# surftemp/cae_tools

Hardware: AMD Instinct MI355X
Metric: train images/sec (16x16->256x256, batch 64) (higher is better)
Workload: dtype f32

## Files before the change

cae_tools_amd/csrc/engine.hip:

```cpp
#include <hip/hip_runtime.h>

#include <dlfcn.h>

#include <algorithm>
#include <cmath>
#include <cstdio>
#include <cstdlib>
#include <cstring>
#include <map>
#include <string>
#include <tuple>
#include <vector>

#include "cae_hip.h"
#include "kernels_generic.h"
#include "kernels_s2.h"
#include "kernels_last.h"
#include "kernels_rows.h"
#include "kernels_gemm.h"
#include "kernels_igemm.h"
#include "kernels_ctlds.h"
#include "kernels_head.h"
#include "dp_comm.h"
#include "kernels_ctbwd.h"
#include "trunk_api.h"
#include "engine_host.h"

namespace cae {
template __global__ void k_ct_fwd_lds<3, 3>(CtFwd);
template __global__ void k_s2_fwd_rows<8, 4, 1, 2>(S2FwdRows);
template __global__ void k_s2_fwd_rows<4, 2, 2, 1>(S2FwdRows);
template __global__ void k_s2_last_fused<2, 1, 4, 4, 4, true, true>(S2Last);
template __global__ void k_s2_bwd_rows<4, 4, 2, 3, 3, 2, 1, 3>(S2Rows);
template __global__ void k_s2_bwd_rows<8, 2, 4, 3, 3, 4, 2, 1>(S2Rows);
}

using namespace cae;
using namespace cae_internal;

namespace cae_internal {
int ctbwd_launch(const void* args, size_t bytes, unsigned gx, unsigned gy, unsigned gz, size_t lds, hipStream_t s);
}

namespace {
thread_local std::string g_err;
}

void cae_detail_set_error(const char* msg) { g_err = msg; }

namespace {

constexpr float kBnEps = 1e-5f;
constexpr float kBnMomentum = 0.1f;
constexpr int kLossSlots = 1 << 16;

// ... 39 lines not shown
    int64_t ws_need = 0;

    float *params = nullptr, *grads = nullptr, *m = nullptr, *v = nullptr, *bufs = nullptr;
    char* ws = nullptr;
    hipStream_t stream = nullptr;
    Hyper hp{1e-3, 0.9, 0.999, 1e-8, 1e-5};
    const float* ds_x[2] = {nullptr, nullptr};
    const float* ds_t[2] = {nullptr, nullptr};
    int64_t ds_n[2] = {0, 0};
    bool graph_mode = true;
    bool lr_stale = true;
    long long captures = 0;
    bool capture_only = false;
    bool use_s2 = true;
    bool variational = false;
    int64_t off_vz = 0, off_vgz = 0, off_zlast = 0;
    cae_internal::TrunkHooks hooks{nullptr, nullptr, nullptr};
    bool gather_fwd = false;
    int ctbwd_mask = 0;
    int ctbwd_auto = 0;
    int64_t off_xbatch = 0;
    bool x_published = false;
    AdamConv0 c0_pending{};
    bool profiling = false;
    struct ProfRec { const char* name; int layer; double bytes; hipEvent_t e0, e1; };
    std::vector<ProfRec> prof;
    std::map<std::tuple<int, int, int, int, const void*, int, int, int, int, int>, hipGraphExec_t> graphs;

    int dp_world = 0, dp_rank = 0;
    RcclApi::comm_t dp_comm = nullptr;
    hipStream_t comm_stream = nullptr;
    hipEvent_t ev_fork = nullptr, ev_join = nullptr;
    bool dp_graph_ok = true;
    bool dp_overlap = true;
    std::vector<int> sync_order;
    size_t sync_pos = 0;
    int64_t bucket_split = 0;

    StepState* state() const { return reinterpret_cast<StepState*>(ws + off_state); }
    double* losses() const { return reinterpret_cast<double*>(ws + off_losses); }
    double* gradacc() const { return reinterpret_cast<double*>(ws + off_gradacc); }
    double* sgacc() const { return reinterpret_cast<double*>(ws + off_sgacc); }
    ShardSegs shard_segs() const {
        ShardSegs r = segs;
        r.base = sgacc();
        return r;
// ... 385 lines not shown
}

void rows_fwd_launch(const ConvLayer& L, S2FwdRows a, hipStream_t s) {
    const RowsPick p = choose_rows_fwd(L);
    a.QH = (L.hout + 1) / 2;
    if (L.cin == 4) rows_fwd_go<4, 2, 2>(a, p.lw, s);
    else rows_fwd_go<8, 4, 1>(a, p.lw, s);
}

bool last_fused_ok(const cae_engine* e, const ConvLayer& L) {
    return s2_eligible(e, L) && L.cin * L.cout * L.kh * L.kw <= 72 && L.sh_b >= 0;
}

constexpr int kLastHB = 4;

struct LastPick { bool vec4, bn; };

int last_strips(const ConvLayer& L) {
    const int qw = (L.wout + 1) / 2;
    const int wmax = L.win > qw - 1 ? L.win : qw - 1;
    return (wmax + kLastStripPx - 1) / kLastStripPx;
}

LastPick choose_last(const ConvLayer& L, bool bn_in) { return LastPick{last_strips(L) == 1 && (L.wout & 3) == 0, bn_in}; }

template <int CIN, int COUT, int KH, int KW>
bool last_fused_launch(S2Last a, LastPick p, hipStream_t s) {
    if constexpr (CIN * COUT * KH * KW <= 72) {
        a.QH = (a.OH + 1) / 2;
        a.QW = (a.OW + 1) / 2;
        const int wmax = a.W > a.QW - 1 ? a.W : a.QW - 1, hmax = a.H > a.QH - 1 ? a.H : a.QH - 1;
        a.strips = (wmax + kLastStripPx - 1) / kLastStripPx;
        a.bands = (hmax + kLastHB - 1) / kLastHB;
        a.total = a.B * a.strips * a.bands;
        const dim3 grid((a.total + 3) / 4);
        if (p.vec4 && p.bn) hipLaunchKernelGGL((k_s2_last_fused<CIN, COUT, KH, KW, kLastHB, true, true>), grid, dim3(256), 0, s, a);
        else if (p.bn) hipLaunchKernelGGL((k_s2_last_fused<CIN, COUT, KH, KW, kLastHB, false, true>), grid, dim3(256), 0, s, a);
        else hipLaunchKernelGGL((k_s2_last_fused<CIN, COUT, KH, KW, kLastHB, false, false>), grid, dim3(256), 0, s, a);
        return true;
    }
    return false;
}

bool last_fused_dispatch(const ConvLayer& L, const S2Last& a, hipStream_t s) {
    const LastPick p = choose_last(L, a.bn_in.mode != BN_NONE);
#define ONE(CI, CO, KH_, KW_) \
    if (L.cin == CI && L.cout == CO && L.kh == KH_ && L.kw == KW_) return last_fused_launch<CI, CO, KH_, KW_>(a, p, s);
#define PAIR(CI, CO) S2_KERNELS(ONE, CI, CO)
    S2_SHAPES(PAIR)
#undef PAIR
#undef ONE
    return false;
}

template <class K>
void head_lds_attr(K kernel, size_t bytes) {
    static size_t granted = 64 * 1024;
    if (bytes > granted) {
// ... 255 lines not shown
    DF_CT_LDS,
    DF_IG,
    DF_UP
};
enum DecBwdK {
    DB_FUSED_LAST,
    DB_ROWS,
    DB_S2,
    DB_CT_LDS,
    DB_IG,
    DB_GENERIC
};

int s2_fwd_epi(const cae_engine* e, int l, bool train, bool external_loss) {
    if (l + 1 < (int)e->dec.size()) return train ? S2_RAW_STATS : S2_RAW;
    if (external_loss) return S2_RAW;
    return train ? S2_SIGMSE : S2_SIGOUT;
}

bool rows_ok(const cae_engine* e, const ConvLayer& L, int l) {
    return l + 1 < (int)e->dec.size() && l > 0 && e->dec[l - 1].has_bn && rows_bwd_ok(e, L);
}

DecFwdK choose_dec_fwd(const cae_engine* e, const ConvLayer& L, int l, int B, bool train, bool external_loss) {
    const bool last = l + 1 == (int)e->dec.size();
    if (last && train && !external_loss && last_fused_ok(e, L)) return DF_FUSED_LAST;
    if (rows_ok(e, L, l)) return DF_ROWS;
    if (s2_eligible(e, L)) return DF_S2;
    if (e->use_s2 && !last && L.stride == 2 && L.kh <= 4 && L.kw <= 4) {
        CtFwd c;
        int waves = 0;
        size_t lds = 0;
        return ct_fwd_plan(e, B, L, l, c, waves, lds) ? DF_CT_LDS : DF_IG;
    }
    return DF_UP;
}

DecBwdK choose_dec_bwd(const cae_engine* e, const ConvLayer& L, int l, int B, bool external_loss) {
    const bool last = l + 1 == (int)e->dec.size();
    if (last && !external_loss && last_fused_ok(e, L)) return DB_FUSED_LAST;
    if (rows_ok(e, L, l)) return DB_ROWS;
    if (s2_eligible(e, L)) return DB_S2;
    if (e->use_s2) {
        CtBwdPlan p;
        return ct_bwd_plan(e, B, L, l, p) ? DB_CT_LDS : DB_IG;
    }
// ... 34 lines not shown
        hipLaunchKernelGGL(k_narrow_range, dim3(grid1(hi - lo)), dim3(256), 0, on, (long long)lo, (long long)hi, e->grads,
                           e->shard_segs(), narrow_tail(e, false, 0));
    }
    if (int rc = dp_allreduce_grads(e, lo, hi, on)) return rc;
    if (overlap) HIP_TRY(hipEventRecord(e->ev_join, e->comm_stream));
    return CAE_OK;
}

int dp_finish_step(cae_engine* e, const StepArgs& a) {
    hipStream_t s = e->stream;
    const int64_t lo = 0, hi = dp_single_collective(e, a) ? e->tab.n_param : e->bucket_split;
    {
        ProfScope _p(e, "dp_narrow_bucket1", 0, 12.0 * (hi - lo));
        hipLaunchKernelGGL(k_narrow_range, dim3(grid1(hi - lo > 0 ? hi - lo : 1)), dim3(256), 0, s, (long long)lo, (long long)hi,
                           e->grads, e->shard_segs(), narrow_tail(e, true, a.inc()));
    }
    if (dp_overlap(e, a)) HIP_TRY(hipStreamWaitEvent(s, e->ev_join, 0));
    if (int rc = dp_allreduce_grads(e, lo, hi, s)) return rc;
    StepTail none;
    memset(&none, 0, sizeof none);
    ProfScope _p(e, "adam", 0, 28.0 * e->tab.n_param);
    hipLaunchKernelGGL(k_adam, dim3(grid1(e->tab.n_param)), dim3(256), 0, s, (long long)e->tab.n_param, e->params,
                       (const float*)e->grads, e->m, e->v, e->hp, (const StepState*)e->state(), e->shard_segs(), none, 0,
                       std::log(e->hp.beta1), std::log(e->hp.beta2), AdamConv0{});
    return CAE_OK;
}

int launch_forward(cae_engine* e, const StepArgs& a) {
    hipStream_t s = e->stream;
    const int B = a.batch;
    const StepState* st = e->state();
    const int act_mode = a.train ? BN_BATCH : BN_RUNNING;

    HeadArgs head;
    size_t head_lds = 0;
    const bool fused_head = a.part == 0 && head_plan(e, a, head, head_lds);
    if (fused_head) {
        head.x = a.x_direct ? a.x_direct : e->ds_x[a.which];
        head.perm = a.x_direct ? nullptr : a.perm;
        head.use_cursor = a.x_direct ? 0 : 1;
        head.bump_adam = a.train ? 1 : 0;
        const int T = (e->fc[3].nout + 15) / 16;
        double bytes = 0;
        for (auto& L : e->enc) bytes += f4((double)B * (L.in_elems() + L.out_elems()));
        for (int i = 0; i < 4; i++) bytes += f4((double)B * (e->fc[i].nin + e->fc[i].nout) + (double)e->fc[i].nin * e->fc[i].nout);
        head_lds_attr(k_head_fwd, head_lds);
        e->x_published = false;
// ... 245 lines not shown
            memset(&f, 0, sizeof f);
            f.B = B; f.H = L.hin; f.W = L.win; f.OH = L.hout; f.OW = L.wout;
            f.in = ain.p;
            f.w = e->params + L.w_off;
            f.bias = e->params + L.b_off;
            f.target = e->ds_t[a.which];
            f.perm = a.perm;
            f.use_cursor = a.use_cursor ? 1 : 0;
            f.st = st;
            f.losses = e->losses();
            f.inv_count = (float)(1.0 / ((double)a.global_batch * L.cout * L.hout * L.wout));
            f.bias_acc = e->sgacc() + L.sh_b;
            f.wacc = e->sgacc() + L.sh_w;
            f.acc_stride = e->segs.n;
            if (l == 0) {
                f.bn_in = bn_none();
                f.gin = e->fptr(e->fc[3].grad_off);
            } else {
                const ConvLayer& P = e->dec[l - 1];
                f.bn_in = bn_of(e, P, BN_BATCH, (double)a.bn_batch * P.hout * P.wout, 1);
                f.gin = e->fptr(P.grad_off);
                f.stats_in = e->bn_stats(P.bn_index);
            }
            ProfScope _p(e, "s2_convt_last_fused", l, f4((double)B * (L.in_elems() * 2.0 + L.out_elems())));
            if (!last_fused_dispatch(L, f, s))
                return fail(CAE_ERR_STATE, "decoder layer %d: no k_s2_last_fused kernel for the chosen variant", (int)l);
            if (l > 0)
                if (int rc = sync_bn_table(e, a, e->dec[l - 1].bn_index)) return rc;
            continue;
        }
        if (bk == DB_ROWS) {
            const ConvLayer& P = e->dec[l - 1];
            S2Rows f;
            memset(&f, 0, sizeof f);
            f.B = B; f.H = L.hin; f.W = L.win; f.OH = L.hout; f.OW = L.wout;
            f.g = gy.p; f.yout = gy.q; f.bn_out = bng;
            f.ain = ain.p; f.bn_in = bna;
            f.w = e->params + L.w_off;
            f.gin = e->fptr(P.grad_off);
            f.stats_in = e->bn_stats(P.bn_index);
            f.wacc = e->sgacc() + L.sh_w;
            f.wacc_stride = e->segs.n;
            f.bg.stats = e->bn_stats(L.bn_index);
            f.bg.gamma_acc = acc + L.gamma_off;
            f.bg.beta_acc = acc + L.beta_off;
            f.bg.C = L.cout;
            f.bg.scale = 1.0 / a.world;
// ... 403 lines not shown
        ProfScope _cal(e, "event_pair", -1, 0.0);
    }
    if (op == OP_DP_TRAIN) {
        e->sync_pos = 0;
        if (a.batch > 0) {
            int rc = launch_forward(e, a);
            if (rc) return rc;
            rc = launch_backward(e, a);
            if (rc) return rc;
        } else {
            hipLaunchKernelGGL(k_bump_adam, dim3(1), dim3(1), 0, s, e->state());
            if (a.dp_sync)
                for (int bn : e->sync_order)
                    if (int rc = sync_bn_table(e, a, bn)) return rc;
            if (int rc = dp_first_bucket(e, a)) return rc;
        }
        if (a.dp_sync && e->sync_pos != e->sync_order.size())
            return fail(CAE_ERR_STATE, "SyncBN: %zu of %zu tables all-reduced", e->sync_pos, e->sync_order.size());
        if (int rc = dp_finish_step(e, a)) return rc;
    } else if (op == OP_TRAIN || op == OP_FWDBWD) {
        StepArgs af = a;
        af.adam_follows = op == OP_TRAIN;
        memset(&e->c0_pending, 0, sizeof e->c0_pending);
        int rc = launch_forward(e, af);
        if (rc) return rc;
        rc = launch_backward(e, af);
        if (rc) return rc;
        if (op == OP_TRAIN) {
            ProfScope _p(e, "adam", 0, 32.0 * e->tab.n_param);
            AdamConv0 c0 = e->c0_pending;
            StepTail tl = step_tail_of(e, a.inc(), 1);
            int nreg = grid1(e->tab.n_param), grid = nreg;
            if (c0.on) {
                const long long skip = (long long)kStatShards * c0.C * 4;
                tl.zero_extra += skip;
                tl.zero_extra_n -= skip;
                c0.n_regular = nreg;
                grid = nreg + c0.nw;
            }
            hipLaunchKernelGGL(k_adam, dim3(grid), dim3(256), 0, s, (long long)e->tab.n_param, e->params,
                               (const float*)nullptr, e->m, e->v, e->hp, (const StepState*)e->state(), e->shard_segs(),
                               tl, 0, std::log(e->hp.beta1), std::log(e->hp.beta2), c0);
        } else {
            hipLaunchKernelGGL(k_acc_to_f32, dim3(grid1(e->tab.n_param)), dim3(256), 0, s, (long long)e->tab.n_param, e->grads,
                               e->shard_segs(), step_tail_of(e, a.inc(), 1));
        }
    } else if (op == OP_EVAL) {
        int rc = launch_forward(e, a);
        if (rc) return rc;
        if (a.use_cursor) hipLaunchKernelGGL(k_advance, dim3(1), dim3(1), 0, s, e->state(), a.inc(), 1, 0);
    } else if (op == OP_ADAM) {
        StepTail none;
        memset(&none, 0, sizeof none);
        hipLaunchKernelGGL(k_adam, dim3(grid1(e->tab.n_param)), dim3(256), 0, s, (long long)e->tab.n_param, e->params,
                           (const float*)e->grads, e->m, e->v, e->hp, (const StepState*)e->state(), e->shard_segs(),
                           none, 0, std::log(e->hp.beta1), std::log(e->hp.beta2), AdamConv0{});
    }
    HIP_TRY(hipGetLastError());
    return CAE_OK;
}

int push_lr(cae_engine* e) {
    if (!e->lr_stale || !e->ws) return CAE_OK;
    hipLaunchKernelGGL(k_set_lr, dim3(1), dim3(1), 0, e->stream, e->state(), e->hp.lr);
    HIP_TRY(hipGetLastError());
    e->lr_stale = false;
    return CAE_OK;
}

int run_op(cae_engine* e, int op, const StepArgs& a, bool cacheable) {
    if (int rc = push_lr(e)) return rc;
    if (!e->graph_mode || !cacheable || e->stream == nullptr || e->profiling)
        return e->capture_only ? CAE_OK : launch_op(e, op, a);
    auto key = std::make_tuple(op, a.which, a.batch, a.global_batch, (const void*)a.perm, a.nsteps, a.cursor_inc,
                               a.dp_sync ? 1 : 0, a.bn_batch, a.world);
    auto it = e->graphs.find(key);
    if (it == e->graphs.end()) {
        hipGraph_t graph = nullptr;
        HIP_TRY(hipStreamBeginCapture(e->stream, hipStreamCaptureModeThreadLocal));
// ... 198 lines not shown
    for (auto& L : e->dec) reg_bn(L);
    e->off_gradacc = carve(e->tab.n_param * (int64_t)sizeof(double));
    e->off_sgacc = carve((int64_t)kStatShards * (e->segs.n > 0 ? e->segs.n : 4) * (int64_t)sizeof(double));
    e->off_zero_end = carve.top;
    for (auto& L : e->enc) e->bn_saved_off[L.bn_index] = carve((int64_t)L.cout * 2 * sizeof(float));
    for (auto& L : e->dec)
        if (L.has_bn) e->bn_saved_off[L.bn_index] = carve((int64_t)L.cout * 2 * sizeof(float));
    const int64_t mb = max_batch;
    for (auto& L : e->enc) {
        L.act_off = carve(mb * L.out_elems() * 4);
        L.grad_off = carve(mb * L.out_elems() * 4);
    }
    for (int i = 0; i < 4; i++) {
        e->fc[i].act_off = carve(mb * e->fc[i].nout * 4);
        e->fc[i].grad_off = carve(mb * e->fc[i].nout * 4);
    }
    for (auto& L : e->dec) {
        if (!L.has_bn) continue;
        L.act_off = carve(mb * L.out_elems() * 4);
        L.grad_off = carve(mb * L.out_elems() * 4);
    }
    e->off_glast = carve(mb * e->dec.back().out_elems() * 4);
    e->off_xbatch = carve((mb * e->enc[0].in_elems() + e->enc[0].cout) * 4);
    if (variational) {
        e->off_vz = carve(mb * latent_size * 4);
        e->off_vgz = carve(mb * latent_size * 4);
        e->off_zlast = carve(mb * e->dec.back().out_elems() * 4);
    }
    e->ws_need = carve.top;
    for (auto& L : e->enc)
        if (L.cin > e->max_channels) e->max_channels = L.cin;
    for (auto& L : e->dec)
        if (L.cin > e->max_channels) e->max_channels = L.cin;
    if (lds_bytes(e->max_channels, e->max_channels) > 60 * 1024) {
        delete e;
        return fail(CAE_ERR_ARG, "channel count %d exceeds the LDS constant table", e->max_channels);
    }
    *out = e;
    return CAE_OK;
}

void cae_engine_destroy(cae_engine* e) {
    if (!e) return;
    e->drop_graphs();
    (void)cae_dp_shutdown(e);
    delete e;
// ... 536 lines not shown
    int n = 0;
    for (auto& r : e->prof) {
        float ms = 0.f;
        hipError_t rc = hipEventElapsedTime(&ms, r.e0, r.e1);
        if (rc == hipSuccess && out && n < capacity) {
            memset(&out[n], 0, sizeof out[n]);
            snprintf(out[n].name, sizeof out[n].name, "%s", r.name);
            out[n].layer = r.layer;
            out[n].micros = (double)ms * 1000.0;
            out[n].bytes = r.bytes;
            n++;
        }
        (void)hipEventDestroy(r.e0);
        (void)hipEventDestroy(r.e1);
    }
    e->prof.clear();
    return n;
}

int cae_debug_plan(const cae_engine* e, int batch, int train, char* out, int64_t out_bytes) {
    if (!e || !out || out_bytes < 1) return fail(CAE_ERR_ARG, "cae_debug_plan: bad argument");
    if (batch < 1 || batch > e->max_batch) return fail(CAE_ERR_ARG, "cae_debug_plan: batch %d outside 1 .. %d", batch, e->max_batch);
    const bool tr = train != 0, ext = e->variational;
    const StepArgs a{0, nullptr, batch, batch, batch, tr, true, nullptr, nullptr, false};
    std::string s;
    char line[256];
    {
        HeadArgs h;
        size_t lds = 0;
        snprintf(line, sizeof line, "head fwd=%s\n", head_plan(e, a, h, lds) ? "fused" : "layers");
        s += line;
    }
    static const char* const kEpiName[] = {"raw_stats", "sigmse", "sigout", "raw"};
    for (int l = 0; l < (int)e->dec.size(); l++) {
        const ConvLayer& L = e->dec[l];
        const int ci = L.cin, co = L.cout, kh = L.kh, kw = L.kw;
        char f[128], b[128];
        switch (choose_dec_fwd(e, L, l, batch, tr, ext)) {
            case DF_FUSED_LAST: {
                const LastPick p = choose_last(L, l > 0 && e->dec[l - 1].has_bn);
                snprintf(f, sizeof f, "last_fused<%d,%d,%d,%d> hb=%d vec4=%d bn=%d", ci, co, kh, kw, kLastHB, (int)p.vec4, (int)p.bn);
                break;
            }
            case DF_ROWS: {
                const RowsPick p = choose_rows_fwd(L);
                snprintf(f, sizeof f, "s2_fwd_rows<%d,%d,%d,%d>", ci, co, p.hb, 64 / p.lw);
                break;
            }
            case DF_S2: {
                const int epi = s2_fwd_epi(e, l, tr, ext);
                const S2FwdPick p = choose_s2_fwd(L, batch, epi);
                const char* fam = p.k == S2F_CS ? "s2_fwd_cs" : (p.k == S2F_QUAD ? "s2_fwd" : "s2_fwd2");
                snprintf(f, sizeof f, "%s<%d,%d,%d,%d,%d> epi=%s", fam, ci, co, kh, kw, p.tw, kEpiName[epi]);
                break;
            }
            case DF_CT_LDS: snprintf(f, sizeof f, "ct_fwd_lds<%d,%d>", kh, kw); break;
            case DF_IG: snprintf(f, sizeof f, "ig_fwd_s2"); break;
            case DF_UP: snprintf(f, sizeof f, "up"); break;
        }
        if (!tr) {
            snprintf(b, sizeof b, "-");
        } else {
            switch (choose_dec_bwd(e, L, l, batch, ext)) {
                case DB_FUSED_LAST: snprintf(b, sizeof b, "(fused)"); break;
// ... 387 lines not shown
    } else if (int rc = launch_forward(e, a)) {
        return rc;
    }
    HIP_TRY(hipGetLastError());
    return CAE_OK;
}

int trunk_backward(cae_engine* e, const float* x, int batch, const ShardSync& sync) {
    if (!e || !e->ws || !e->variational) return fail(CAE_ERR_STATE, "trunk_backward: not a bound trunk engine");
    StepArgs a = trunk_args(x, batch, true, sync);
    a.external_loss = true;
    if (int rc = batch == 0 ? trunk_empty_shard(e, a, false) : launch_backward(e, a)) return rc;
    if (a.ordered && e->sync_pos != e->sync_order.size())
        return fail(CAE_ERR_STATE, "SyncBN: %zu of %zu tables passed to the callback", e->sync_pos, e->sync_order.size());
    HIP_TRY(hipGetLastError());
    return CAE_OK;
}

int trunk_adam(cae_engine* e) {
    if (!e || !e->ws) return fail(CAE_ERR_STATE, "trunk_adam: not a bound engine");
    if (int rc = push_lr(e)) return rc;
    hipLaunchKernelGGL(k_adam, dim3(grid1(e->tab.n_param)), dim3(256), 0, e->stream, (long long)e->tab.n_param, e->params,
                       (const float*)nullptr, e->m, e->v, e->hp, (const StepState*)e->state(), e->shard_segs(),
                       step_tail_of(e, 0, 0), 0, std::log(e->hp.beta1), std::log(e->hp.beta2), AdamConv0{});
    HIP_TRY(hipGetLastError());
    return CAE_OK;
}

int trunk_gradients(cae_engine* e, float* out, double scale) {
    if (!e || !e->ws || !out) return fail(CAE_ERR_STATE, "trunk_gradients: bad argument");
    hipLaunchKernelGGL(k_acc_to_f32, dim3(grid1(e->tab.n_param)), dim3(256), 0, e->stream, (long long)e->tab.n_param, out, e->shard_segs(),
                       step_tail_of(e, 0, 0));
    if (scale != 1.0)
        hipLaunchKernelGGL(k_scale_f32, dim3(grid1(e->tab.n_param)), dim3(256), 0, e->stream, out, (long long)e->tab.n_param, (float)scale);
    HIP_TRY(hipGetLastError());
    return CAE_OK;
}

int trunk_adam_from(cae_engine* e, const float* grads) {
    if (!e || !e->ws || !grads) return fail(CAE_ERR_STATE, "trunk_adam_from: bad argument");
    if (int rc = push_lr(e)) return rc;
    StepTail none;
    memset(&none, 0, sizeof none);
    hipLaunchKernelGGL(k_adam, dim3(grid1(e->tab.n_param)), dim3(256), 0, e->stream, (long long)e->tab.n_param, e->params, grads, e->m, e->v,
                       e->hp, (const StepState*)e->state(), e->shard_segs(), none, 0, std::log(e->hp.beta1), std::log(e->hp.beta2),
                       AdamConv0{});
    HIP_TRY(hipGetLastError());
    return CAE_OK;
}

}
```

cae_tools_amd/csrc/kernels_generic.h:

```cpp
#pragma once
#include <hip/hip_runtime.h>
#include <stdint.h>

namespace cae {

constexpr int kStatShards = 8;

#include "acc_grid.h"

struct ShardSeg {
    long long param_off;
    int count;
    int sh_off;
};
struct ShardSegs {
    int nseg;
    int n;
    const double* base;
    ShardSeg seg[12];
};

__device__ __forceinline__ double sharded_grad(const ShardSegs& ss, long long i) {
    double g = 0.0;
    for (int s = 0; s < ss.nseg; s++) {
// ... 678 lines not shown
    float sum = 0.f, bsum = 0.f;
    for (int b = 0; b < B; b++) {
        const float gv = gout[(size_t)b * nout + o];
        sum = fmaf(gv, bn_apply(bni.mode, k, in[(size_t)b * nin + i], 0.f), sum);
        bsum += gv;
    }
    accW[idx] = (double)sum;
    if (i == 0) accB[o] = (double)bsum;
}

struct Hyper {
    double lr, beta1, beta2, eps, wd;
};

struct StepTail {
    double* zero_extra;
    long long zero_extra_n;
    double* acc_rw;
    double* shard_rw;
    StepState* st;
    int batch_inc, slot_inc;
};

__device__ __forceinline__ float consume_grad(const StepTail& tl, const ShardSegs& ss, long long i) {
    double g = tl.acc_rw[i];
    tl.acc_rw[i] = 0.0;
    for (int s = 0; s < ss.nseg; s++) {
        const long long d = i - ss.seg[s].param_off;
        if (d >= 0 && d < ss.seg[s].count) {
            double* p = tl.shard_rw + ss.seg[s].sh_off + d;
            double v[kStatShards];
#pragma unroll
            for (int sh = 0; sh < kStatShards; sh++) v[sh] = p[(size_t)sh * ss.n];
#pragma unroll
            for (int sh = 0; sh < kStatShards; sh++) {
                g += v[sh];
                p[(size_t)sh * ss.n] = 0.0;
            }
        }
    }
    return (float)g;
}

__device__ __forceinline__ void step_tail(const StepTail& tl, long long gid, long long nthreads) {
    for (long long j = gid; j < tl.zero_extra_n; j += nthreads) tl.zero_extra[j] = 0.0;
    if (gid == 0 && tl.st) {
        tl.st->batch_start += tl.batch_inc;
        tl.st->loss_slot += tl.slot_inc;
    }
}

struct AdamConv0 {
    int on, nw, C, n_regular;
    long long w_off, gamma_off, beta_off;
    ConvGeom g;
    Src small;
    BnDesc bns;
    const float* xb;
    const double* stats;
    double scale;
};
constexpr int kAdamConv0Pos = 16;

__device__ __forceinline__ void adam_conv0_body(const AdamConv0& c0, float* __restrict__ p, float* __restrict__ m,
// ... 45 lines not shown
    const float4 ks = cs4[cs];
    float sum = 0.f;
#pragma unroll
    for (int u = 0; u < kAdamConv0Pos; u++)
        if (tid + u * 256 < n) sum = fmaf(bn_apply(BN_BWD, ks, sp[u], sq[u]), lp[u], sum);
    for (int pp = tid + kAdamConv0Pos * 256; pp < n; pp += 256) {
        float a, b, c;
        fetch(pp, a, b, c);
        sum = fmaf(bn_apply(BN_BWD, ks, a, b), c, sum);
    }
    const double tot = block_sum((double)sum, red);
    if (tid == 0) {
        float gr = (float)(tot * c0.scale);
        if (h.wd != 0.0) gr = fmaf((float)h.wd, w, gr);
        mi = mi + (gr - mi) * (float)(1.0 - h.beta1);
        vi = vi * (float)h.beta2 + ((float)(1.0 - h.beta2) * gr) * gr;
        const float denom = sqrtf(vi) / corr[1] + (float)h.eps;
        p[pi] = w - corr[0] * (mi / denom);
        m[pi] = mi;
        v[pi] = vi;
    }
}

__global__ void __launch_bounds__(256) k_adam(long long n, float* __restrict__ p, const float* __restrict__ g32,
                                               float* __restrict__ m, float* __restrict__ v, Hyper h,
                                               const StepState* __restrict__ st, ShardSegs ss, StepTail tl, int t_add,
                                               double ln_b1, double ln_b2, AdamConv0 c0) {
    kernarg_warm<sizeof(Hyper) + sizeof(ShardSegs) + sizeof(StepTail) + 72 + sizeof(AdamConv0)>();
    const long long i = (long long)blockIdx.x * 256 + threadIdx.x;
    __shared__ float corr[2];
    if (c0.on && (int)blockIdx.x >= c0.n_regular) {
        __shared__ double red0[8];
        __shared__ float4 cs40[64];
        adam_conv0_body(c0, p, m, v, h, st, t_add, ln_b1, ln_b2, corr, red0, cs40);
        return;
    }
    for (long long j = i; j < tl.zero_extra_n; j += (long long)(c0.on ? c0.n_regular : (int)gridDim.x) * 256) tl.zero_extra[j] = 0.0;
    int t = 0;
    double lr = 0.0;
    if (threadIdx.x < 2) {
        optimiser_state(st, t, lr);
        t += t_add;
    }
    const bool moves_cursor = i == 0 && tl.st != nullptr;
    long long cursor = 0;
    int slot = 0;
    if (moves_cursor) {
        cursor = tl.st->batch_start;
        slot = tl.st->loss_slot;
    }
    const bool mine = i < n && !(c0.on && i >= c0.w_off && i < c0.w_off + c0.nw);
    float g = 0.f, w = 0.f, mi = 0.f, vi = 0.f;
    double gacc = 0.0, sv[kStatShards], bv[kStatShards];
    double* shp = nullptr;
    const double* bnp = nullptr;
    if (mine) {
        w = p[i];
        mi = m[i];
        vi = v[i];
        if (g32) {
            g = g32[i];
        } else {
            gacc = tl.acc_rw[i];
            for (int sg = 0; sg < ss.nseg; sg++) {
                const long long d = i - ss.seg[sg].param_off;
                if (d >= 0 && d < ss.seg[sg].count) shp = tl.shard_rw + ss.seg[sg].sh_off + d;
            }
            if (shp) {
#pragma unroll
                for (int sh = 0; sh < kStatShards; sh++) sv[sh] = shp[(size_t)sh * ss.n];
            }
            if (c0.on) {
                const long long dg = i - c0.gamma_off, db = i - c0.beta_off;
                if (dg >= 0 && dg < c0.C) bnp = c0.stats + dg * 4 + 3;
// ... 556 lines not shown
```

cae_tools_amd/csrc/kernels_last.h:

```cpp
#pragma once
#include <utility>
#include "kernels_s2.h"

namespace cae {

template <class F, int... Is>
__device__ __forceinline__ void static_for_impl(F&& f, std::integer_sequence<int, Is...>) {
    (f(std::integral_constant<int, Is>{}), ...);
}
template <int N, class F>
__device__ __forceinline__ void static_for(F&& f) {
    static_for_impl(f, std::make_integer_sequence<int, N>{});
}

struct S2Last {
    int B, H, W, OH, OW;
    int QH, QW;
    int strips, bands;
    int total;
    const float* in;
    BnDesc bn_in;
    const float* w;
    const float* bias;
    const float* target;
    const int* perm;
    int use_cursor;
    const StepState* st;
    double* losses;
    float inv_count;
    double* bias_acc;
    double* wacc;
    int acc_stride;
    float* gin;
    double* stats_in;
};

constexpr int kLastStripPx = 127;

__device__ __forceinline__ float uniform_f(float v) {
    return __builtin_bit_cast(float, __builtin_amdgcn_readfirstlane(__builtin_bit_cast(int, v)));
}
__device__ __forceinline__ float from_left(float v, float edge) {
    return __builtin_bit_cast(float, __builtin_amdgcn_update_dpp(__builtin_bit_cast(int, edge), __builtin_bit_cast(int, v), 0x138, 0xF, 0xF, false));
}
__device__ __forceinline__ float from_right(float v, float edge) {
    return __builtin_bit_cast(float, __builtin_amdgcn_update_dpp(__builtin_bit_cast(int, edge), __builtin_bit_cast(int, v), 0x130, 0xF, 0xF, false));
}

constexpr int kWsumLd = 68;
constexpr int kWsumScratch = 16 * kWsumLd;
template <int N>
__device__ __forceinline__ void wave_sums_lds(const float (&v)[N], float* scr, float* out, int lane) {
    const int row = lane >> 2, qd = lane & 3;
#pragma unroll
    for (int c0 = 0; c0 < N; c0 += 16) {
#pragma unroll
        for (int i = 0; i < 16; i++)
            if (c0 + i < N) scr[i * kWsumLd + lane] = v[c0 + i];
        const float4* p = reinterpret_cast<const float4*>(scr + row * kWsumLd + 4 * qd);
        const float4 a0 = p[0], a1 = p[4], a2 = p[8], a3 = p[12];
        float t = ((a0.x + a0.y) + (a0.z + a0.w)) + ((a1.x + a1.y) + (a1.z + a1.w)) + ((a2.x + a2.y) + (a2.z + a2.w)) +
                  ((a3.x + a3.y) + (a3.z + a3.w));
        t += dpp_f<0xB1>(t);
        t += dpp_f<0x4E>(t);
        if (qd == 0 && c0 + row < N) out[c0 + row] = t;
    }
}

template <int CIN, int COUT, int KH, int KW, int HB, bool VEC4, bool BN>
__global__ void __launch_bounds__(256) __attribute__((amdgpu_waves_per_eu(1, 2))) k_s2_last_fused(S2Last a) {
    kernarg_warm<sizeof(S2Last)>();
    constexpr int NACC = CIN * COUT * KH * KW;
    constexpr int NRED = NACC + 2 * CIN;
    constexpr int NR = HB + 1;
    static_assert(KH >= 3 && KH <= 4 && KW >= 3 && KW <= 4, "3- or 4-tap stride-2 kernels");
    __shared__ float redf[4 * NRED];
    __shared__ double redd[4 * 2 * COUT];
    __shared__ __attribute__((aligned(16))) float wscr[4 * kWsumScratch];
    __shared__ float xch[4 * CIN * 2 * 64];

    const int tid = threadIdx.x, lane = tid & 63;
    const int wv = __builtin_amdgcn_readfirstlane(tid >> 6);
    const unsigned HW = a.H * a.W, OHW = a.OH * a.OW;

    const int item = blockIdx.x * 4 + wv;
    const bool work = item < a.total;
    const int it = work ? item : 0;
    const int b = it / (a.strips * a.bands);
    const int rem = it - b * (a.strips * a.bands);
    const int band = rem / a.strips, strip = rem - band * a.strips;
    const int m0 = band * HB;
    const bool last_band = band == a.bands - 1, last_strip = strip == a.strips - 1;
// ... 303 lines not shown
        if (y < a.H) {
            const bool p0 = n0 < a.W, p1 = n0 + 1 < a.W && lane < 63;
#pragma unroll
            for (int ci = 0; ci < CIN; ci++) {
                float gv0 = carry[ci][0] + xch[(((wv + 1) * CIN + ci) * 2 + 0) * 64 + lane];
                float gv1 = carry[ci][1] + xch[(((wv + 1) * CIN + ci) * 2 + 1) * 64 + lane];
                if constexpr (BN) {
                    const float e0 = rin[HB][ci][0] - kc[ci].x, e1 = rin[HB][ci][1] - kc[ci].x;
                    gv0 = fmaf(e0, kc[ci].y, kc[ci].z) > 0.f ? gv0 : 0.f;
                    gv1 = fmaf(e1, kc[ci].y, kc[ci].z) > 0.f ? gv1 : 0.f;
                    const float s0 = p0 ? gv0 : 0.f, s1 = p1 ? gv1 : 0.f;
                    d1[ci] += s0 + s1;
                    d2[ci] = fmaf(s0, e0 * kc[ci].w, fmaf(s1, e1 * kc[ci].w, d2[ci]));
                }
                float* gp = a.gin + (size_t)(b * CIN + ci) * HW + (unsigned)y * a.W + n0;
                if (p0) {
                    gp[0] = gv0;
                    gp[p1 ? 1 : 0] = p1 ? gv1 : gv0;
                }
            }
        }
    }

    {
        float red[NRED];
#pragma unroll
        for (int i = 0; i < NACC; i++) red[i] = dw[i];
#pragma unroll
        for (int c = 0; c < CIN; c++) {
            red[NACC + 2 * c] = d1[c];
            red[NACC + 2 * c + 1] = d2[c];
        }
        wave_sums_lds<NRED>(red, wscr + wv * kWsumScratch, redf + wv * NRED, lane);
    }
#pragma unroll
    for (int co = 0; co < COUT; co++) {
        const double t1 = wave_sum_lane63((double)ls[co] * (double)a.inv_count), t2 = wave_sum_lane63((double)gs[co]);
        if (lane == 63) {
            redd[(wv * COUT + co) * 2] = t1;
            redd[(wv * COUT + co) * 2 + 1] = t2;
        }
    }
    __syncthreads();
    const int shard = blockIdx.x & (kStatShards - 1);
    for (int j = tid; j < NRED + 2 * COUT; j += 256) {
        if (j < NRED) {
            const double s = (double)redf[j] + (double)redf[NRED + j] + (double)redf[2 * NRED + j] + (double)redf[3 * NRED + j];
            if (j < NACC) {
                acc_add<ACC_GRAD>(&a.wacc[(size_t)shard * a.acc_stride + j], s);
            } else if (a.stats_in) {
                const int jj = j - NACC;
                acc_add<ACC_GRAD>(&a.stats_in[((size_t)shard * CIN + (jj >> 1)) * 4 + 2 + (jj & 1)], s);
            }
        } else {
            const int q = j - NRED, co = q >> 1, which = q & 1;
            double s = 0.0;
#pragma unroll
            for (int w = 0; w < 4; w++) s += redd[(w * COUT + co) * 2 + which];
            if (which == 0) acc_add<ACC_GRAD>(&a.losses[(size_t)loss_slot_v * kStatShards + shard], s);
            else acc_add<ACC_GRAD>(&a.bias_acc[(size_t)shard * a.acc_stride + co], s);
        }
    }
    asm volatile("" :: "v"(perm_val_v));
}

}
```

cae_tools_amd/engine.py:

```python
import ctypes as C
from collections import OrderedDict

import numpy as np
import torch

from . import _lib
from ._engine_base import TEST, TRAIN, SpecPlan, _spec_layers, _to_c, require_gpu
from ._lib import CaeError, check


class EnginePlan(SpecPlan):

    PREFIX = "cae_"

    def bn_prefixes(self):
        return [n[: -len(".running_mean")] for n in self.tensors if n.endswith(".running_mean")]

    def set_kernel_mode(self, mode):
        check(self.lib.cae_set_kernel_mode(self.handle, int(mode)))

    def kernel_plan(self, batch, train):
        buf = C.create_string_buffer(1 << 16)
        check(self.lib.cae_debug_plan(self.handle, int(batch), 1 if train else 0, buf, len(buf)))
        plan = {}
        for line in buf.value.decode().splitlines():
            (name, *fields) = line.split()
            plan[name] = dict(f.split("=", 1) for f in fields)
        return plan


class HipEngine(EnginePlan):

    def __init__(self, spec, fc_size, latent_size, max_batch, device=None, graph=True, specialised=True):
        require_gpu()
        super().__init__(spec, fc_size, latent_size, max_batch)
        self._bind(device, grads=True, buffers=True)
        check(self.lib.cae_set_graph_mode(self.handle, 1 if graph else 0))
        check(self.lib.cae_set_kernel_mode(self.handle, int(specialised) if isinstance(specialised, int) and not isinstance(specialised, bool) else (1 if specialised else 0)))
        torch.cuda.synchronize(self.device)
        self.num_batches_tracked = 0
        self.adam_steps = 0
        self._datasets = {}
        self._keep = []
        self.loss_slots = int(self.lib.cae_loss_slots(self.handle))
        self._slot = 0
        self._cursor = None
# ... 574 lines not shown
```

Baseline: 384,100.

## Write last-layer weight/bias/loss partial sums to a slab reduced inside Adam

In the fused last decoder kernel, each block now writes its weight-gradient, bias-gradient and loss partial sums to a per-block row in a double-precision slab instead of issuing sharded atomic adds. The Adam kernel gains extra blocks that reduce the slab columns and apply the update for those parameters directly, and it also accumulates the loss. This is meant to remove atomic contention on the small last-layer gradient set. The cost is extra slab memory traffic, extra Adam blocks, and a code path that only applies to single-device fused training steps.

```diff
diff --git a/cae_tools_amd/csrc/engine.hip b/cae_tools_amd/csrc/engine.hip
--- a/cae_tools_amd/csrc/engine.hip
+++ b/cae_tools_amd/csrc/engine.hip
@@ -31,6 +31,7 @@
 template __global__ void k_s2_fwd_rows<8, 4, 1, 2>(S2FwdRows);
 template __global__ void k_s2_fwd_rows<4, 2, 2, 1>(S2FwdRows);
 template __global__ void k_s2_last_fused<2, 1, 4, 4, 4, true, true>(S2Last);
+template __global__ void k_s2_last_fused<2, 1, 4, 4, 4, true, true, true>(S2Last);
 template __global__ void k_s2_bwd_rows<4, 4, 2, 3, 3, 2, 1, 3>(S2Rows);
 template __global__ void k_s2_bwd_rows<8, 2, 4, 3, 3, 4, 2, 1>(S2Rows);
 }
@@ -116,6 +117,9 @@
     int64_t off_xbatch = 0;
     bool x_published = false;
     AdamConv0 c0_pending{};
+    int64_t off_slab_last = 0;
+    int slab_last_rows = 0;
+    AdamSlab slab_pending{};
     bool profiling = false;
     struct ProfRec { const char* name; int layer; double bytes; hipEvent_t e0, e1; };
     std::vector<ProfRec> prof;
@@ -547,6 +551,13 @@
     return (wmax + kLastStripPx - 1) / kLastStripPx;
 }
 
+int last_grid(const ConvLayer& L, int B) {
+    const int qh = (L.hout + 1) / 2;
+    const int hmax = L.hin > qh - 1 ? L.hin : qh - 1;
+    const int bands = (hmax + kLastHB - 1) / kLastHB;
+    return (B * last_strips(L) * bands + 3) / 4;
+}
+
 LastPick choose_last(const ConvLayer& L, bool bn_in) { return LastPick{last_strips(L) == 1 && (L.wout & 3) == 0, bn_in}; }
 
 template <int CIN, int COUT, int KH, int KW>
@@ -559,6 +570,13 @@
         a.bands = (hmax + kLastHB - 1) / kLastHB;
         a.total = a.B * a.strips * a.bands;
         const dim3 grid((a.total + 3) / 4);
+        if (a.slab) {
+            a.slab_stride = last_slab_stride(CIN * COUT * KH * KW, COUT);
+            if (p.vec4 && p.bn) hipLaunchKernelGGL((k_s2_last_fused<CIN, COUT, KH, KW, kLastHB, true, true, true>), grid, dim3(256), 0, s, a);
+            else if (p.bn) hipLaunchKernelGGL((k_s2_last_fused<CIN, COUT, KH, KW, kLastHB, false, true, true>), grid, dim3(256), 0, s, a);
+            else hipLaunchKernelGGL((k_s2_last_fused<CIN, COUT, KH, KW, kLastHB, false, false, true>), grid, dim3(256), 0, s, a);
+            return true;
+        }
         if (p.vec4 && p.bn) hipLaunchKernelGGL((k_s2_last_fused<CIN, COUT, KH, KW, kLastHB, true, true>), grid, dim3(256), 0, s, a);
         else if (p.bn) hipLaunchKernelGGL((k_s2_last_fused<CIN, COUT, KH, KW, kLastHB, false, true>), grid, dim3(256), 0, s, a);
         else hipLaunchKernelGGL((k_s2_last_fused<CIN, COUT, KH, KW, kLastHB, false, false>), grid, dim3(256), 0, s, a);
@@ -860,6 +878,10 @@
     return l + 1 < (int)e->dec.size() && l > 0 && e->dec[l - 1].has_bn && rows_bwd_ok(e, L);
 }
 
+bool last_slab(const cae_engine* e, const StepArgs& a) {
+    return a.adam_follows && !a.syncing() && a.world == 1 && !a.dp && !a.external_loss && e->slab_last_rows > 0;
+}
+
 DecFwdK choose_dec_fwd(const cae_engine* e, const ConvLayer& L, int l, int B, bool train, bool external_loss) {
     const bool last = l + 1 == (int)e->dec.size();
     if (last && train && !external_loss && last_fused_ok(e, L)) return DF_FUSED_LAST;
@@ -940,7 +962,7 @@
     ProfScope _p(e, "adam", 0, 28.0 * e->tab.n_param);
     hipLaunchKernelGGL(k_adam, dim3(grid1(e->tab.n_param)), dim3(256), 0, s, (long long)e->tab.n_param, e->params,
                        (const float*)e->grads, e->m, e->v, e->hp, (const StepState*)e->state(), e->shard_segs(), none, 0,
-                       std::log(e->hp.beta1), std::log(e->hp.beta2), AdamConv0{});
+                       std::log(e->hp.beta1), std::log(e->hp.beta2), AdamConv0{}, AdamSlab{});
     return CAE_OK;
 }
 
@@ -1232,7 +1254,24 @@
                 f.gin = e->fptr(P.grad_off);
                 f.stats_in = e->bn_stats(P.bn_index);
             }
-            ProfScope _p(e, "s2_convt_last_fused", l, f4((double)B * (L.in_elems() * 2.0 + L.out_elems())));
+            double slab_bytes = 0.0;
+            if (last_slab(e, a)) {
+                const int nw = L.cin * L.cout * L.kh * L.kw, rows = last_grid(L, B);
+                if (rows > e->slab_last_rows)
+                    return fail(CAE_ERR_STATE, "decoder layer %d: %d slab rows, the arena holds %d", (int)l, rows, e->slab_last_rows);
+                f.slab = reinterpret_cast<double*>(e->ws + e->off_slab_last);
+                AdamSlab& sl = e->slab_pending;
+                memset(&sl, 0, sizeof sl);
+                sl.on = 1;
+                sl.nrows = rows;
+                sl.stride = last_slab_stride(nw, L.cout);
+                sl.nw = nw; sl.nb = L.cout; sl.nl = 1;
+                sl.w_off = L.w_off; sl.b_off = L.b_off;
+                sl.rows = f.slab;
+                sl.losses = e->losses();
+                slab_bytes = 8.0 * rows * (nw + L.cout + 2);
+            }
+            ProfScope _p(e, "s2_convt_last_fused", l, f4((double)B * (L.in_elems() * 2.0 + L.out_elems())) + slab_bytes);
             if (!last_fused_dispatch(L, f, s))
                 return fail(CAE_ERR_STATE, "decoder layer %d: no k_s2_last_fused kernel for the chosen variant", (int)l);
             if (l > 0)
@@ -1682,13 +1721,15 @@
         StepArgs af = a;
         af.adam_follows = op == OP_TRAIN;
         memset(&e->c0_pending, 0, sizeof e->c0_pending);
+        memset(&e->slab_pending, 0, sizeof e->slab_pending);
         int rc = launch_forward(e, af);
         if (rc) return rc;
         rc = launch_backward(e, af);
         if (rc) return rc;
         if (op == OP_TRAIN) {
-            ProfScope _p(e, "adam", 0, 32.0 * e->tab.n_param);
             AdamConv0 c0 = e->c0_pending;
+            AdamSlab sl = e->slab_pending;
+            ProfScope _p(e, "adam", 0, 32.0 * e->tab.n_param + (sl.on ? 8.0 * sl.nrows * (sl.nw + sl.nb + sl.nl) : 0.0));
             StepTail tl = step_tail_of(e, a.inc(), 1);
             int nreg = grid1(e->tab.n_param), grid = nreg;
             if (c0.on) {
@@ -1698,9 +1739,14 @@
                 c0.n_regular = nreg;
                 grid = nreg + c0.nw;
             }
+            if (sl.on) {
+                sl.n_regular = nreg;
+                sl.first_block = grid;
+                grid += (sl.nw + sl.nb + sl.nl + kAdamSlabVals - 1) / kAdamSlabVals;
+            }
             hipLaunchKernelGGL(k_adam, dim3(grid), dim3(256), 0, s, (long long)e->tab.n_param, e->params,
                                (const float*)nullptr, e->m, e->v, e->hp, (const StepState*)e->state(), e->shard_segs(),
-                               tl, 0, std::log(e->hp.beta1), std::log(e->hp.beta2), c0);
+                               tl, 0, std::log(e->hp.beta1), std::log(e->hp.beta2), c0, sl);
         } else {
             hipLaunchKernelGGL(k_acc_to_f32, dim3(grid1(e->tab.n_param)), dim3(256), 0, s, (long long)e->tab.n_param, e->grads,
                                e->shard_segs(), step_tail_of(e, a.inc(), 1));
@@ -1714,7 +1760,7 @@
         memset(&none, 0, sizeof none);
         hipLaunchKernelGGL(k_adam, dim3(grid1(e->tab.n_param)), dim3(256), 0, s, (long long)e->tab.n_param, e->params,
                            (const float*)e->grads, e->m, e->v, e->hp, (const StepState*)e->state(), e->shard_segs(),
-                           none, 0, std::log(e->hp.beta1), std::log(e->hp.beta2), AdamConv0{});
+                           none, 0, std::log(e->hp.beta1), std::log(e->hp.beta2), AdamConv0{}, AdamSlab{});
     }
     HIP_TRY(hipGetLastError());
     return CAE_OK;
@@ -1959,6 +2005,14 @@
     }
     e->off_glast = carve(mb * e->dec.back().out_elems() * 4);
     e->off_xbatch = carve((mb * e->enc[0].in_elems() + e->enc[0].cout) * 4);
+    {
+        const ConvLayer& L = e->dec.back();
+        const int nw = L.cin * L.cout * L.kh * L.kw;
+        if (L.sh_b >= 0 && s2_shape_ok(L) && nw <= 72) {
+            e->slab_last_rows = last_grid(L, max_batch);
+            e->off_slab_last = carve((int64_t)e->slab_last_rows * last_slab_stride(nw, L.cout) * (int64_t)sizeof(double));
+        }
+    }
     if (variational) {
         e->off_vz = carve(mb * latent_size * 4);
         e->off_vgz = carve(mb * latent_size * 4);
@@ -2541,7 +2595,8 @@
     if (!e || !out || out_bytes < 1) return fail(CAE_ERR_ARG, "cae_debug_plan: bad argument");
     if (batch < 1 || batch > e->max_batch) return fail(CAE_ERR_ARG, "cae_debug_plan: batch %d outside 1 .. %d", batch, e->max_batch);
     const bool tr = train != 0, ext = e->variational;
-    const StepArgs a{0, nullptr, batch, batch, batch, tr, true, nullptr, nullptr, false};
+    StepArgs a{0, nullptr, batch, batch, batch, tr, true, nullptr, nullptr, false};
+    a.adam_follows = train == 2;
     std::string s;
     char line[256];
     {
@@ -2558,7 +2613,8 @@
         switch (choose_dec_fwd(e, L, l, batch, tr, ext)) {
             case DF_FUSED_LAST: {
                 const LastPick p = choose_last(L, l > 0 && e->dec[l - 1].has_bn);
-                snprintf(f, sizeof f, "last_fused<%d,%d,%d,%d> hb=%d vec4=%d bn=%d", ci, co, kh, kw, kLastHB, (int)p.vec4, (int)p.bn);
+                int at = snprintf(f, sizeof f, "last_fused<%d,%d,%d,%d> hb=%d vec4=%d bn=%d", ci, co, kh, kw, kLastHB, (int)p.vec4, (int)p.bn);
+                if (train >= 2) snprintf(f + at, sizeof f - at, " sums=%s", last_slab(e, a) ? "slab" : "atomics");
                 break;
             }
             case DF_ROWS: {
@@ -2992,7 +3048,7 @@
     if (int rc = push_lr(e)) return rc;
     hipLaunchKernelGGL(k_adam, dim3(grid1(e->tab.n_param)), dim3(256), 0, e->stream, (long long)e->tab.n_param, e->params,
                        (const float*)nullptr, e->m, e->v, e->hp, (const StepState*)e->state(), e->shard_segs(),
-                       step_tail_of(e, 0, 0), 0, std::log(e->hp.beta1), std::log(e->hp.beta2), AdamConv0{});
+                       step_tail_of(e, 0, 0), 0, std::log(e->hp.beta1), std::log(e->hp.beta2), AdamConv0{}, AdamSlab{});
     HIP_TRY(hipGetLastError());
     return CAE_OK;
 }
@@ -3014,7 +3070,7 @@
     memset(&none, 0, sizeof none);
     hipLaunchKernelGGL(k_adam, dim3(grid1(e->tab.n_param)), dim3(256), 0, e->stream, (long long)e->tab.n_param, e->params, grads, e->m, e->v,
                        e->hp, (const StepState*)e->state(), e->shard_segs(), none, 0, std::log(e->hp.beta1), std::log(e->hp.beta2),
-                       AdamConv0{});
+                       AdamConv0{}, AdamSlab{});
     HIP_TRY(hipGetLastError());
     return CAE_OK;
 }
diff --git a/cae_tools_amd/csrc/kernels_generic.h b/cae_tools_amd/csrc/kernels_generic.h
--- a/cae_tools_amd/csrc/kernels_generic.h
+++ b/cae_tools_amd/csrc/kernels_generic.h
@@ -724,7 +724,7 @@
     int batch_inc, slot_inc;
 };
 
-__device__ __forceinline__ float consume_grad(const StepTail& tl, const ShardSegs& ss, long long i) {
+__device__ __forceinline__ double consume_grad_f64(const StepTail& tl, const ShardSegs& ss, long long i) {
     double g = tl.acc_rw[i];
     tl.acc_rw[i] = 0.0;
     for (int s = 0; s < ss.nseg; s++) {
@@ -741,7 +741,10 @@
             }
         }
     }
-    return (float)g;
+    return g;
+}
+__device__ __forceinline__ float consume_grad(const StepTail& tl, const ShardSegs& ss, long long i) {
+    return (float)consume_grad_f64(tl, ss, i);
 }
 
 __device__ __forceinline__ void step_tail(const StepTail& tl, long long gid, long long nthreads) {
@@ -833,20 +836,93 @@
     }
 }
 
+struct AdamSlab {
+    int on, n_regular, first_block;
+    int nrows, stride;
+    int nw, nb, nl;
+    long long w_off, b_off;
+    const double* rows;
+    double* losses;
+};
+constexpr int kAdamSlabVals = 8, kAdamSlabLanes = 256 / kAdamSlabVals;
+
+__device__ __forceinline__ void adam_slab_body(const AdamSlab& sl, float* __restrict__ p, float* __restrict__ m,
+                                               float* __restrict__ v, const Hyper& h, const StepState* __restrict__ st,
+                                               const ShardSegs& ss, const StepTail& tl, int t_add, double ln_b1, double ln_b2,
+                                               float* corr, double* part) {
+    const int tid = threadIdx.x, e = tid & (kAdamSlabVals - 1), rl = tid / kAdamSlabVals;
+    const int j = ((int)blockIdx.x - sl.first_block) * kAdamSlabVals + e;
+    const int npar = sl.nw + sl.nb, nval = npar + sl.nl;
+    const bool live = j < nval, owner = live && rl == 0;
+    int t = 0;
+    double lr = 0.0;
+    if (tid < 2) {
+        optimiser_state(st, t, lr);
+        t += t_add;
+    }
+    const bool is_par = owner && j < npar;
+    const long long pi = j < sl.nw ? sl.w_off + j : sl.b_off + (j - sl.nw);
+    float w = 0.f, mi = 0.f, vi = 0.f;
+    double gacc = 0.0, slot_d = 0.0;
+    if (is_par) {
+        w = p[pi];
+        mi = m[pi];
+        vi = v[pi];
+        gacc = consume_grad_f64(tl, ss, pi);
+    } else if (owner) {
+        slot_d = sl.rows[nval];
+    }
+    double acc = 0.0;
+    if (live) {
+        const double* col = sl.rows + j;
+#pragma unroll 8
+        for (int r = rl; r < sl.nrows; r += kAdamSlabLanes) acc += col[(size_t)r * sl.stride];
+    }
+    part[tid] = acc;
+    if (tid < 2) {
+        const double bc = -expm1((double)t * (tid ? ln_b2 : ln_b1));
+        corr[tid] = tid ? (float)sqrt(bc) : (float)(lr / bc);
+    }
+    __syncthreads();
+#pragma unroll
+    for (int half = kAdamSlabLanes / 2; half >= 1; half >>= 1) {
+        if (rl < half) part[tid] += part[tid + half * kAdamSlabVals];
+        __syncthreads();
+    }
+    if (is_par) {
+        float g = (float)(gacc + part[tid]);
+        if (h.wd != 0.0) g = fmaf((float)h.wd, w, g);
+        mi = mi + (g - mi) * (float)(1.0 - h.beta1);
+        vi = vi * (float)h.beta2 + ((float)(1.0 - h.beta2) * g) * g;
+        const float denom = sqrtf(vi) / corr[1] + (float)h.eps;
+        p[pi] = w - corr[0] * (mi / denom);
+        m[pi] = mi;
+        v[pi] = vi;
+    } else if (owner) {
+        sl.losses[(size_t)(int)slot_d * kStatShards] += part[tid];
+    }
+}
+
 __global__ void __launch_bounds__(256) k_adam(long long n, float* __restrict__ p, const float* __restrict__ g32,
                                                float* __restrict__ m, float* __restrict__ v, Hyper h,
                                                const StepState* __restrict__ st, ShardSegs ss, StepTail tl, int t_add,
-                                               double ln_b1, double ln_b2, AdamConv0 c0) {
-    kernarg_warm<sizeof(Hyper) + sizeof(ShardSegs) + sizeof(StepTail) + 72 + sizeof(AdamConv0)>();
+                                               double ln_b1, double ln_b2, AdamConv0 c0, AdamSlab sl) {
+    kernarg_warm<sizeof(Hyper) + sizeof(ShardSegs) + sizeof(StepTail) + 72 + sizeof(AdamConv0) + sizeof(AdamSlab)>();
     const long long i = (long long)blockIdx.x * 256 + threadIdx.x;
     __shared__ float corr[2];
+    if (sl.on && (int)blockIdx.x >= sl.first_block) {
+        __shared__ double part[256];
+        adam_slab_body(sl, p, m, v, h, st, ss, tl, t_add, ln_b1, ln_b2, corr, part);
+        return;
+    }
     if (c0.on && (int)blockIdx.x >= c0.n_regular) {
         __shared__ double red0[8];
         __shared__ float4 cs40[64];
         adam_conv0_body(c0, p, m, v, h, st, t_add, ln_b1, ln_b2, corr, red0, cs40);
         return;
     }
-    for (long long j = i; j < tl.zero_extra_n; j += (long long)(c0.on ? c0.n_regular : (int)gridDim.x) * 256) tl.zero_extra[j] = 0.0;
+    const int n_regular = c0.on ? c0.n_regular : sl.on ? sl.n_regular : (int)gridDim.x;
+    for (long long j = i; j < tl.zero_extra_n; j += (long long)n_regular * 256) tl.zero_extra[j] = 0.0;
     int t = 0;
     double lr = 0.0;
     if (threadIdx.x < 2) {
@@ -860,7 +936,8 @@
         cursor = tl.st->batch_start;
         slot = tl.st->loss_slot;
     }
-    const bool mine = i < n && !(c0.on && i >= c0.w_off && i < c0.w_off + c0.nw);
+    const bool mine = i < n && !(c0.on && i >= c0.w_off && i < c0.w_off + c0.nw) &&
+                      !(sl.on && ((i >= sl.w_off && i < sl.w_off + sl.nw) || (i >= sl.b_off && i < sl.b_off + sl.nb)));
     float g = 0.f, w = 0.f, mi = 0.f, vi = 0.f;
     double gacc = 0.0, sv[kStatShards], bv[kStatShards];
     double* shp = nullptr;
diff --git a/cae_tools_amd/csrc/kernels_last.h b/cae_tools_amd/csrc/kernels_last.h
--- a/cae_tools_amd/csrc/kernels_last.h
+++ b/cae_tools_amd/csrc/kernels_last.h
@@ -33,7 +33,11 @@
     int acc_stride;
     float* gin;
     double* stats_in;
+    double* slab;
+    int slab_stride;
 };
+
+constexpr int last_slab_stride(int nacc, int cout) { return (nacc + cout + 2 + 15) / 16 * 16; }
 
 constexpr int kLastStripPx = 127;
 
@@ -67,7 +71,7 @@
     }
 }
 
-template <int CIN, int COUT, int KH, int KW, int HB, bool VEC4, bool BN>
+template <int CIN, int COUT, int KH, int KW, int HB, bool VEC4, bool BN, bool SLAB = false>
 __global__ void __launch_bounds__(256) __attribute__((amdgpu_waves_per_eu(1, 2))) k_s2_last_fused(S2Last a) {
     kernarg_warm<sizeof(S2Last)>();
     constexpr int NACC = CIN * COUT * KH * KW;
@@ -417,7 +421,25 @@
         }
     }
 
-    {
+    const int shard = blockIdx.x & (kStatShards - 1);
+    if constexpr (SLAB) {
+        if constexpr (BN) {
+            float red[2 * CIN];
+#pragma unroll
+            for (int c = 0; c < CIN; c++) {
+                red[2 * c] = d1[c];
+                red[2 * c + 1] = d2[c];
+            }
+            wave_sums_lds<2 * CIN>(red, wscr + wv * kWsumScratch, redf + wv * NRED + NACC, lane);
+            __syncthreads();
+            if (tid < 2 * CIN && a.stats_in) {
+                const int j = NACC + tid;
+                const double s = (double)redf[j] + (double)redf[NRED + j] + (double)redf[2 * NRED + j] + (double)redf[3 * NRED + j];
+                acc_add<ACC_GRAD>(&a.stats_in[((size_t)shard * CIN + (tid >> 1)) * 4 + 2 + (tid & 1)], s);
+            }
+        }
+        wave_sums_lds<NACC>(dw, wscr + wv * kWsumScratch, redf + wv * NRED, lane);
+    } else {
         float red[NRED];
 #pragma unroll
         for (int i = 0; i < NACC; i++) red[i] = dw[i];
@@ -437,8 +459,33 @@
         }
     }
     __syncthreads();
-    const int shard = blockIdx.x & (kStatShards - 1);
-    for (int j = tid; j < NRED + 2 * COUT; j += 256) {
+    if constexpr (SLAB) {
+        constexpr int NROW = NACC + COUT + 1;
+        static_assert(NROW + 1 <= 256, "one thread per row entry");
+        double* row = a.slab + (size_t)blockIdx.x * a.slab_stride;
+        if (tid < NACC) {
+            row[tid] = (double)redf[tid] + (double)redf[NRED + tid] + (double)redf[2 * NRED + tid] + (double)redf[3 * NRED + tid];
+        } else if (tid < NACC + COUT) {
+            const int co = tid - NACC;
+            double s = 0.0;
+#pragma unroll
+            for (int w = 0; w < 4; w++) s += redd[(w * COUT + co) * 2 + 1];
+            row[tid] = s;
+        } else if (tid == NACC + COUT) {
+            double s = 0.0;
+#pragma unroll
+            for (int co = 0; co < COUT; co++) {
+                double sc = 0.0;
+#pragma unroll
+                for (int w = 0; w < 4; w++) sc += redd[(w * COUT + co) * 2];
+                s += sc;
+            }
+            row[tid] = s;
+        } else if (tid == NROW) {
+            row[tid] = (double)loss_slot_v;
+        }
+    }
+    for (int j = tid; !SLAB && j < NRED + 2 * COUT; j += 256) {
         if (j < NRED) {
             const double s = (double)redf[j] + (double)redf[NRED + j] + (double)redf[2 * NRED + j] + (double)redf[3 * NRED + j];
             if (j < NACC) {
diff --git a/cae_tools_amd/engine.py b/cae_tools_amd/engine.py
--- a/cae_tools_amd/engine.py
+++ b/cae_tools_amd/engine.py
@@ -19,9 +19,10 @@
     def set_kernel_mode(self, mode):
         check(self.lib.cae_set_kernel_mode(self.handle, int(mode)))
 
-    def kernel_plan(self, batch, train):
+    def kernel_plan(self, batch, train, step=None):
         buf = C.create_string_buffer(1 << 16)
-        check(self.lib.cae_debug_plan(self.handle, int(batch), 1 if train else 0, buf, len(buf)))
+        mode = {None: 1, "fused": 2, "split": 3}[step] if train else 0
+        check(self.lib.cae_debug_plan(self.handle, int(batch), mode, buf, len(buf)))
         plan = {}
         for line in buf.value.decode().splitlines():
             (name, *fields) = line.split()
```

After: 387,700 (median of 6 runs). About the same (+0.9%).
